# AUTOMATIC1111/stable-diffusion-webui

Measured on AMD Instinct MI355X. Metric: images/sec SD1.5 512x512 20-step Euler-a, batch 8 per GPU, higher is better.
Workload: dtype f16

## Files before the change

stable-diffusion-webui_amd/csrc/attention.hip:

```cpp
#include "common.h"
#include "prof.h"
#include <cstdlib>

namespace sdmi {

typedef float f2v __attribute__((ext_vector_type(2)));
typedef unsigned u4v __attribute__((ext_vector_type(4)));

__device__ __forceinline__ float max3f(float a, float b, float c) { return fmaxf(fmaxf(a, b), c); }
template <int NKB>
__device__ __forceinline__ float tree_max(const f16v (&sc)[NKB]) {
    constexpr int N = NKB * 16;
    float v[N];
#pragma unroll
    for (int i = 0; i < N; ++i) v[i] = sc[i >> 4][i & 15];
    int n = N;
#pragma unroll
    for (int level = 0; level < 6; ++level) {
        if (n <= 1) break;
        const int m = (n + 2) / 3;
#pragma unroll
        for (int i = 0; i < m; ++i) {
            const int a = 3 * i, b = a + 1 < n ? a + 1 : a, c = a + 2 < n ? a + 2 : a;
            v[i] = max3f(v[a], v[b], v[c]);
// ... 413 lines not shown
    h8 qf[NDC];
    {
        const half_t* qptr = p.q + ((long)b * p.N + (qok ? q : 0)) * p.ldq + h * D;
#pragma unroll
        for (int dc = 0; dc < NDC; ++dc) {
            const int d = dc * 16 + half * 8;
            h8 v = {0, 0, 0, 0, 0, 0, 0, 0};
            if (qok && d < D) v = *reinterpret_cast<const h8*>(qptr + d);
            if constexpr (FOLD) {
#pragma unroll
                for (int j = 0; j < 8; ++j) v[j] = (half_t)((float)v[j] * fold_p2(p.scale_log2));
            }
            qf[dc] = v;
        }
    }
    const half_t* kbase = p.k + (long)b * p.M * p.ldk + h * D;
    const half_t* vbase = p.vt + ((long)b * p.H + h) * D * (long)p.vt_ld;

    u4v kr[K_IT], vr[V_IT];
    auto load_k = [&](int key0) {
#pragma unroll
        for (int it = 0; it < K_IT; ++it) {
            const int idx = it * NT + tid;
            const int row = idx / KCR, c = idx - row * KCR;
            const int rr = min(key0 + row, p.M - 1);
            kr[it] = *reinterpret_cast<const u4v*>(kbase + (long)rr * p.ldk + c * 8);
        }
    };
    auto load_v = [&](int key0) {
#pragma unroll
        for (int it = 0; it < V_IT; ++it) {
            const int idx = it * NT + tid;
            const int row = idx / VCPR, c = idx - row * VCPR;
            const int col = min(key0 + c * 8, p.vt_ld - 8);
            vr[it] = *reinterpret_cast<const u4v*>(vbase + (long)min(row, D - 1) * p.vt_ld + col);
        }
    };
    char* const dump = smem + NSLOT * SLOT + K_BYTES + tid * 16;
    auto write_k = [&](char* Ks) {
#pragma unroll
        for (int it = 0; it < K_IT; ++it) {
            const int idx = it * NT + tid;
            const int row = idx / KCR, c = idx - row * KCR;
            char* dst = (KCH % NT == 0 || idx < KCH) ? Ks + row * KSTR + c * 16 : dump;
            *reinterpret_cast<u4v*>(dst) = kr[it];
        }
    };
    auto write_v = [&](char* Vs) {
#pragma unroll
        for (int it = 0; it < V_IT; ++it) {
            const int idx = it * NT + tid;
            const int row = idx / VCPR, c = idx - row * VCPR;
            char* dst = (VCH % NT == 0 || idx < VCH) ? Vs + row * VSTR + c * 16 : dump;
            *reinterpret_cast<u4v*>(dst) = vr[it];
        }
    };
    auto section_barrier = [&](bool wait_lds = true) {
        __builtin_amdgcn_sched_barrier(0);
        if (wait_lds) asm volatile("s_waitcnt lgkmcnt(0)" ::: "memory");
        __builtin_amdgcn_s_barrier();
        asm volatile("" ::: "memory");
        __builtin_amdgcn_sched_barrier(0);
    };

    const int T = (p.M + KVT - 1) / KVT;
    const int nfull = p.M / KVT;
    char* const K0s = smem + NSLOT * SLOT;

    {
        constexpr int KPAD = KCPR - KCR;
        if constexpr (KPAD > 0) {
            for (int i = tid; i < (NSLOT + 1) * KVT * KPAD; i += NT) {
                const int img = i / (KVT * KPAD), j = i - img * (KVT * KPAD);
                const int row = j / KPAD, c = KCR + j % KPAD;
                char* base = img < NSLOT ? smem + img * SLOT : K0s;
                const unsigned w0 = (FOLD && c == KCR) ? 0x00003C00u : 0u;
                *reinterpret_cast<uint4*>(base + row * KSTR + c * 16) = make_uint4(w0, 0u, 0u, 0u);
            }
        }
        if constexpr (SUMROW) {
            constexpr int PADCH = (DV - D) * VCPR;
            for (int i = tid; i < NSLOT * PADCH; i += NT) {
                const int img = i / PADCH, j = i - img * PADCH;
                const int row = D + j / VCPR, c = j % VCPR;
                const unsigned w = row == D ? 0x3C003C00u : 0u;
                *reinterpret_cast<uint4*>(smem + img * SLOT + K_BYTES + row * VSTR + c * 16) = make_uint4(w, w, w, w);
            }
        }
        load_k(0);
        write_k(K0s);
        load_v(0); load_k(KVT);
        write_v(smem + K_BYTES); write_k(smem);
        if (T > 1) {
            load_v(KVT); load_k(2 * KVT);
            write_v(smem + SLOT + K_BYTES); write_k(smem + SLOT);
        }
    }
    asm volatile("s_waitcnt lgkmcnt(0)" ::: "memory");
    __builtin_amdgcn_s_barrier();
    asm volatile("" ::: "memory");

    const int krow = (lq & 0x13) | ((lq & 4) << 1) | ((lq & 8) >> 1);
    const int ka_off = krow * KSTR + half * 16;
    const int va_off = K_BYTES + lq * VSTR + half * 16;

    f16v o[NDB], sc[NKB];
#pragma unroll
    for (int db = 0; db < NDB; ++db)
#pragma unroll
        for (int r = 0; r < 16; ++r) o[db][r] = 0.f;
#pragma unroll
    for (int kb = 0; kb < NKB; ++kb)
#pragma unroll
        for (int r = 0; r < 16; ++r) sc[kb][r] = 0.f;
    {
        h8 kaf0[NDC][NKB];
#pragma unroll
        for (int dc = 0; dc < NDC; ++dc)
#pragma unroll
            for (int kb = 0; kb < NKB; ++kb) kaf0[dc][kb] = *reinterpret_cast<const h8*>(K0s + ka_off + kb * 32 * KSTR + dc * 32);
#pragma unroll
        for (int dc = 0; dc < NDC; ++dc)
#pragma unroll
            for (int kb = 0; kb < NKB; ++kb) sc[kb] = __builtin_amdgcn_mfma_f32_32x32x16_f16(kaf0[dc][kb], qf[dc], sc[kb], 0, 0, 0);
    }
    load_v(2 * KVT); load_k(3 * KVT);

    float shift = FOLD ? 0.f : -1e30f;
    f2v l_run = {0.f, 0.f};
    const f2v sl2 = {p.scale_log2, p.scale_log2};
    [[maybe_unused]] const float fr = p.scale_log2 / fold_p2(p.scale_log2);
    [[maybe_unused]] const f2v fr2 = {fr, fr};
    h8 pb[NKB][2];
    h8 kaf[NDC][NKB], vaf[NDB][NKB][2];

    section_barrier();
    for (int i = 0; i < grp; ++i) section_barrier();
    constexpr int NB = NG;

    for (int t = 0; t < T; ++t) {
        const long long ta = stamp();
        long long tb = ta, tc = ta;
        if (t >= nfull || p.causal) {
            asm volatile("");
            int lim = p.M - t * KVT - 8 * half;
            if (p.causal) lim = min(lim, q + 1 - t * KVT - 8 * half);
#pragma unroll
            for (int kb = 0; kb < NKB; ++kb)
#pragma unroll
                for (int r = 0; r < 16; ++r)
                    if (32 * kb + 16 * (r >> 3) + (r & 7) >= lim) sc[kb][r] = -INFINITY;
        }
        float mx = tree_max<NKB>(sc);
        {
            float mlo = mx, mhi = mx;
            asm volatile("s_nop 1\n\tv_permlane32_swap_b32 %0, %1" : "+v"(mlo), "+v"(mhi));
            mx = fmaxf(mlo, mhi);
        }
        if constexpr (FOLD) {
            const bool raise = t == 0 || __builtin_amdgcn_ballot_w64(mx > 0.f) != 0;
            if (raise) {
                asm volatile("");
                const float want = shift + mx;
                const float ns = (t == 0 || mx > 0.f) ? (float)(half_t)fminf(fmaxf(want, -60000.f), 60000.f) : shift;
                const float delta = ns - shift;
                shift = ns;
                if (t > 0) {
                    const float alpha = __builtin_amdgcn_exp2f(-delta * fr);
#pragma unroll
                    for (int db = 0; db < NDB; ++db)
#pragma unroll
                        for (int r = 0; r < 16; ++r) o[db][r] *= alpha;
                    if (!SUMROW) l_run = l_run * alpha;
                }
#pragma unroll
                for (int kb = 0; kb < NKB; ++kb)
#pragma unroll
                    for (int r = 0; r < 16; ++r) sc[kb][r] -= delta;
                if (half == PHALF) qf[PDC][0] = (half_t)(-ns);
            }
        } else {
            mx *= p.scale_log2;
            const float m_new = fmaxf(shift, mx);
            const float alpha = __builtin_amdgcn_exp2f(shift - m_new);
            const bool moved = __builtin_amdgcn_ballot_w64(m_new > shift) != 0;
            shift = m_new;
            if (!SUMROW) l_run = l_run * alpha;
            if (moved) {
#pragma unroll
                for (int db = 0; db < NDB; ++db)
#pragma unroll
                    for (int r = 0; r < 16; ++r) o[db][r] *= alpha;
            }
        }
        const f2v mneg = {-shift, -shift};
        auto exp_block = [&](int kb) {
            f2v rs = {0.f, 0.f};
#pragma unroll
            for (int r = 0; r < 16; r += 2) {
                f2v e;
                if constexpr (FOLD) {
                    const f2v y = f2v{sc[kb][r], sc[kb][r + 1]} * fr2;
                    e = f2v{__builtin_amdgcn_exp2f(y.x), __builtin_amdgcn_exp2f(y.y)};
                } else {
                    const f2v s2 = {sc[kb][r], sc[kb][r + 1]};
                    const f2v y = __builtin_elementwise_fma(s2, sl2, mneg);
                    e = f2v{__builtin_amdgcn_exp2f(y.x), __builtin_amdgcn_exp2f(y.y)};
                }
                if (!SUMROW) rs += e;
                pb[kb][r >> 3][r & 7] = (half_t)e.x;
                pb[kb][r >> 3][(r & 7) + 1] = (half_t)e.y;
            }
            if (!SUMROW) l_run += rs;
        };
        auto bar = [&](int k, bool wait_lds) {
            if (!(t + 1 == T && k >= NB - grp)) section_barrier(wait_lds);
        };
        exp_block(0);
        if constexpr (NG == 3) {
            asm volatile("" :: "v"(pb[0][0]), "v"(pb[0][1]));
            tb = stamp();
            bar(0, false);
            tc = stamp();
        }
#pragma unroll
        for (int kb = 1; kb < NKB; ++kb) exp_block(kb);
        {
            const char* tile = smem + (t % NSLOT) * SLOT;
#pragma unroll
            for (int db = 0; db < NDB; ++db)
#pragma unroll
                for (int kb = 0; kb < NKB; ++kb)
#pragma unroll
                    for (int sb = 0; sb < 2; ++sb)
                        vaf[db][kb][sb] = *reinterpret_cast<const h8*>(tile + va_off + db * 32 * VSTR + (kb * 32 + sb * 16) * 2);
#pragma unroll
            for (int dc = 0; dc < NDC; ++dc)
#pragma unroll
                for (int kb = 0; kb < NKB; ++kb) kaf[dc][kb] = *reinterpret_cast<const h8*>(tile + ka_off + kb * 32 * KSTR + dc * 32);
        }
#pragma unroll
        for (int kb = 0; kb < NKB; ++kb) asm volatile("" :: "v"(pb[kb][0]), "v"(pb[kb][1]));
        const long long td = stamp();
        bar(NB - 2, false);
        const long long te = stamp();
#pragma unroll
        for (int kb = 0; kb < NKB; ++kb)
#pragma unroll
            for (int r = 0; r < 16; ++r) sc[kb][r] = 0.f;
        {
            char* slot = smem + ((t + 2) % NSLOT) * SLOT;
            write_v(slot + K_BYTES); write_k(slot);
            load_v((t + 3) * KVT); load_k((t + 4) * KVT);
        }
#pragma unroll
        for (int step = 0; step < (NDC > 2 * NKB ? NDC : 2 * NKB); ++step) {
            if (step < 2 * NKB) {
                const int kb = step >> 1, sb = step & 1;
#pragma unroll
                for (int db = 0; db < NDB; ++db) o[db] = __builtin_amdgcn_mfma_f32_32x32x16_f16(vaf[db][kb][sb], pb[kb][sb], o[db], 0, 0, 0);
            }
            if (step < NDC) {
#pragma unroll
                for (int kb = 0; kb < NKB; ++kb) sc[kb] = __builtin_amdgcn_mfma_f32_32x32x16_f16(kaf[step][kb], qf[step], sc[kb], 0, 0, 0);
            }
        }
        const long long tf = stamp();
        bar(NB - 1, true);
        if constexpr (TIMING) {
            const long long tg = stamp();
            tm[0] += tb - ta; tm[1] += tc - tb; tm[2] += td - tc; tm[3] += te - td; tm[4] += tf - te; tm[5] += tg - tf; tm[6] += 1;
        }
    }
    if constexpr (TIMING) {
        if (p.dbg && lane == 0) {
            long long* dst = p.dbg + ((long)(blockIdx.y * gridDim.x + blockIdx.x) * (4 * NG) + wave) * 8;
#pragma unroll
            for (int i = 0; i < 7; ++i) dst[i] = tm[i];
        }
    }

    float l_tot;
    if (SUMROW) l_tot = __shfl(o[L_DB][L_R], lq + 32 * L_HALF);
    else l_tot = (l_run.x + l_run.y) + __shfl_xor(l_run.x + l_run.y, 32);
    const float inv = 1.0f / l_tot;
    if (qok) {
        half_t* optr = p.out + ((long)b * p.N + q) * p.ldo + h * D;
#pragma unroll
        for (int db = 0; db < NDB; ++db) {
#pragma unroll
            for (int g = 0; g < 4; ++g) {
                const int d0 = db * 32 + g * 8 + half * 4;
                if (d0 < D) {
                    h4 v;
#pragma unroll
                    for (int e = 0; e < 4; ++e) v[e] = (half_t)(o[db][g * 4 + e] * inv);
                    *reinterpret_cast<h4*>(optr + d0) = v;
                }
            }
        }
    }
}

__global__ __launch_bounds__(64) void attn_generic_kernel(AttnP p) {
    extern __shared__ float sc[];
    const int lane = threadIdx.x;
    const int q = blockIdx.x, bh = blockIdx.y, b = bh / p.H, h = bh - b * p.H;
    const half_t* qptr = p.q + ((long)b * p.N + q) * p.ldq + h * p.D;
    const half_t* kbase = p.k + (long)b * p.M * p.ldk + h * p.D;
    const half_t* vbase = p.vt + ((long)b * p.H + h) * p.D * (long)p.vt_ld;
    float mx = -INFINITY;
    const int m_vis = p.causal ? min(p.M, q + 1) : p.M;
    for (int key = lane; key < p.M; key += 64) {
        if (key >= m_vis) { sc[key] = -INFINITY; continue; }
        const half_t* kp = kbase + (long)key * p.ldk;
        float acc = 0.f;
        for (int d = 0; d < p.D; ++d) acc = fmaf((float)qptr[d], (float)kp[d], acc);
        acc *= p.scale_log2;
        sc[key] = acc;
        mx = fmaxf(mx, acc);
    }
    for (int off = 32; off > 0; off >>= 1) mx = fmaxf(mx, __shfl_xor(mx, off));
    float sum = 0.f;
    for (int key = lane; key < p.M; key += 64) {
        const float e = exp2f(sc[key] - mx);
        sc[key] = e;
        sum += e;
    }
    for (int off = 32; off > 0; off >>= 1) sum += __shfl_xor(sum, off);
    __syncthreads();
    const float inv = 1.0f / sum;
    for (int d = lane; d < p.D; d += 64) {
        const half_t* vp = vbase + (long)d * p.vt_ld;
        float acc = 0.f;
        for (int key = 0; key < p.M; ++key) acc = fmaf(sc[key], (float)vp[key], acc);
        p.out[((long)b * p.N + q) * p.ldo + h * p.D + d] = (half_t)(acc * inv);
    }
}

__global__ __launch_bounds__(256) void transpose_v_kernel(const half_t* v, half_t* vt, int M, int C, int ldv, int Mpad) {
    __shared__ half_t tile[32][33];
    const int b = blockIdx.z;
    const int m0 = blockIdx.x * 32, c0 = blockIdx.y * 32;
    const int tx = threadIdx.x & 31, ty = threadIdx.x >> 5;
    for (int i = ty; i < 32; i += 8) {
        const int m = m0 + i, c = c0 + tx;
        tile[i][tx] = (m < M && c < C) ? v[((long)b * M + m) * ldv + c] : (half_t)0;
    }
    __syncthreads();
    for (int i = ty; i < 32; i += 8) {
        const int c = c0 + i, m = m0 + tx;
        if (c < C && m < Mpad) vt[((long)b * C + c) * Mpad + m] = tile[tx][i];
    }
}

int launch_transpose_v(const half_t* v, half_t* vt, int B, int H, int M, int D, int ldv, int Mpad, hipStream_t s) {
    const int C = H * D;
    dim3 grid(cdiv(Mpad, 32), cdiv(C, 32), B);
    hipLaunchKernelGGL(transpose_v_kernel, grid, dim3(256), 0, s, v, vt, M, C, ldv, Mpad);
    SDMI_CHECK_HIP(hipGetLastError());
    return 0;
}

unsigned long long g_attn_dbg = 0;
int g_attn_kvt = [] { const char* e = getenv("SDMI_ATTN_KVT"); return e ? atoi(e) : 0; }();

int g_attn_occ = [] { const char* e = getenv("SDMI_ATTN_OCC"); return e ? atoi(e) : 15; }();
int g_attn_tau = [] { const char* e = getenv("SDMI_ATTN_TAU"); return e ? atoi(e) : 8; }();
int g_attn_fold_min_m = [] { const char* e = getenv("SDMI_ATTN_FOLD_MIN_M"); return e ? atoi(e) : 1024; }();
int g_attn_lds_pad = 0;
int g_attn_pp_min_m = [] { const char* e = getenv("SDMI_ATTN_PP_MIN_M"); return e ? atoi(e) : 256; }();

template <int D, int KVT, int VAR = 0>
static int launch_attn_d(const AttnP& p, hipStream_t s) {
    constexpr int DK = (D + 15) / 16 * 16, DV = (D + 31) / 32 * 32;
    constexpr int SMEM = 2 * (KVT * (DK * 2 + 16) + DV * (KVT * 2 + 16));
    auto kern = attn_mfma_kernel<D, KVT, VAR>;
    static PerDeviceOnce attr;
    const int smem = SMEM + (g_attn_lds_pad > 0 ? g_attn_lds_pad : 0);
    if (attr.need(smem)) SDMI_CHECK_HIP(hipFuncSetAttribute((const void*)kern, hipFuncAttributeMaxDynamicSharedMemorySize, smem));
    dim3 grid(cdiv(p.N, 128), p.B * p.H);
    hipLaunchKernelGGL(kern, grid, dim3(256), smem, s, p);
    SDMI_CHECK_HIP(hipGetLastError());
    return 0;
}

template <int D, bool FOLD, int NG = 2, bool TIMING = false>
static int launch_attn_pp(const AttnP& p, hipStream_t s) {
    constexpr int DK = (D + 15) / 16 * 16, DV = (D + 31) / 32 * 32;
    constexpr int SMEM = 3 * (64 * (DK * 2 + 16) + DV * (64 * 2 + 16)) + 64 * (DK * 2 + 16) + NG * 256 * 16;
    auto kern = attn_pp_kernel<D, FOLD, NG, TIMING>;
    static PerDeviceOnce attr;
    if (attr.need()) SDMI_CHECK_HIP(hipFuncSetAttribute((const void*)kern, hipFuncAttributeMaxDynamicSharedMemorySize, SMEM));
    dim3 grid(cdiv(p.N, NG * 128), p.B * p.H);
    hipLaunchKernelGGL(kern, grid, dim3(NG * 256), SMEM, s, p);
    SDMI_CHECK_HIP(hipGetLastError());
    return 0;
}

int launch_attention(const AttnP& p_in, bool force_generic, hipStream_t s) {
    AttnP p = p_in;
    p.tau = (float)(g_attn_tau < 0 ? -1 : g_attn_tau > 12 ? 12 : g_attn_tau);
    SDMI_REQUIRE(p.B > 0 && p.H > 0 && p.N > 0 && p.M > 0 && p.D > 0, "empty attention");
    SDMI_REQUIRE(p.vt_ld >= (p.M + 63) / 64 * 64, "vt_ld must be >= M rounded up to 64");
    const double pf_flops = 4.0 * p.B * p.H * (double)p.N * p.M * p.D;
    const double pf_bytes = 2.0 * p.B * p.H * ((double)p.N * p.D * 2 + (double)p.M * p.D * 2);
    ProfScope ps(force_generic ? "attention_generic" : (p.M > 128 ? "attention_mfma_self" : "attention_mfma_cross"), pf_flops, pf_bytes, s);
    const bool aligned = (p.ldq % 8 == 0) && (p.ldk % 8 == 0) && (p.vt_ld % 8 == 0) && (p.ldo % 4 == 0) && (p.D % 8 == 0);
    const bool kvt128 = g_attn_kvt == 128;
    if (!force_generic && aligned) {
        if (g_attn_kvt == 96 && p.M > 64 && p.M <= 96 && !p.causal) {
            switch (p.D) {
                case 40: return launch_attn_d<40, 96, 0>(p, s);
                case 64: return launch_attn_d<64, 96>(p, s);
                case 80: return launch_attn_d<80, 96>(p, s);
                case 160: return launch_attn_d<160, 96>(p, s);
                default: break;
            }
        }
        switch (p.D) {
            case 40:
                if ((g_attn_occ == 20 || g_attn_occ == 21) && p.M >= g_attn_pp_min_m && p.N >= 256)
                    return g_attn_occ == 21 ? launch_attn_pp<40, true>(p, s) : launch_attn_pp<40, false>(p, s);
                if ((g_attn_occ == 28 || g_attn_occ == 38) && p.M >= g_attn_pp_min_m && p.N >= 384) {
                    AttnP q = p; q.dbg = (long long*)g_attn_dbg;
                    return g_attn_occ == 38 ? launch_attn_pp<40, true, 3, true>(q, s) : launch_attn_pp<40, true, 2, true>(q, s);
                }
                if ((g_attn_occ == 30 || g_attn_occ == 31) && p.M >= g_attn_pp_min_m && p.N >= 384)
                    return g_attn_occ == 31 ? launch_attn_pp<40, true, 3>(p, s) : launch_attn_pp<40, false, 3>(p, s);
                if (!(kvt128 && p.M > 64)) {
                    if (g_attn_occ == 5) return launch_attn_d<40, 64, 5>(p, s);
                    if (g_attn_occ == 15 && g_attn_fold_min_m > 0 && p.M >= g_attn_fold_min_m && p.N >= g_attn_fold_min_m && !p.causal)
                        return launch_attn_d<40, 64, 17>(p, s);
                    if (g_attn_occ == 15) return launch_attn_d<40, 64, 15>(p, s);
                    if (g_attn_occ == 16) return launch_attn_d<40, 64, 16>(p, s);
                    if (g_attn_occ == 17) return launch_attn_d<40, 64, 17>(p, s);
#ifdef SDMI_ATTN_PARTS
                    if (g_attn_occ == 10) return launch_attn_d<40, 64, 10>(p, s);
                    if (g_attn_occ == 11) return launch_attn_d<40, 64, 11>(p, s);
                    if (g_attn_occ == 12) return launch_attn_d<40, 64, 12>(p, s);
                    if (g_attn_occ == 13) return launch_attn_d<40, 64, 13>(p, s);
                    if (g_attn_occ == 14) return launch_attn_d<40, 64, 14>(p, s);
                    if (g_attn_occ == 18) { AttnP q = p; q.dbg = (long long*)g_attn_dbg; return launch_attn_d<40, 64, 18>(q, s); }
#endif
                }
                return (kvt128 && p.M > 64) ? launch_attn_d<40, 128>(p, s) : launch_attn_d<40, 64>(p, s);
            case 64:
                if ((g_attn_occ == 20 || g_attn_occ == 21) && p.M >= g_attn_pp_min_m && p.N >= 256) return launch_attn_pp<64, false>(p, s);
                return (kvt128 && p.M > 64) ? launch_attn_d<64, 128>(p, s) : launch_attn_d<64, 64>(p, s);
            case 80: return launch_attn_d<80, 64>(p, s);
            case 128: return launch_attn_d<128, 64>(p, s);
            case 160: return launch_attn_d<160, 64>(p, s);
            default: break;
        }
    }
    SDMI_REQUIRE(p.D <= 512 && p.M <= 16384, "generic attention supports D <= 512 and M <= 16384");
    static PerDeviceOnce attr;
    if (attr.need()) SDMI_CHECK_HIP(hipFuncSetAttribute((const void*)attn_generic_kernel, hipFuncAttributeMaxDynamicSharedMemorySize, 16384 * 4));
    hipLaunchKernelGGL(attn_generic_kernel, dim3(p.N, p.B * p.H), dim3(64), p.M * sizeof(float), s, p);
    SDMI_CHECK_HIP(hipGetLastError());
    return 0;
}

}
```

stable-diffusion-webui_amd/csrc/capi.cpp:

```cpp
#include "engine.h"
#include "prof.h"
#include <cstring>

namespace sdmi {
extern int g_vae_attn_rows;
int unet_forward(sdmi_engine* e, const void* x, const void* t, const void* ctx, const void* y, void* out, int io_dtype,
                 int Bn, int h, int w, int L, hipStream_t s);
int vae_decode(sdmi_engine* e, const void* z, int io_dtype, float* out, int B, int h, int w, hipStream_t s);
int vae_encode(sdmi_engine* e, const void* x, int io_dtype, float* out, int B, int H, int W, hipStream_t s);
int engine_load_unet_tensor(sdmi_engine* e, const char* key, const void* data, int dtype, int ndim, const int64_t* shape, int on_device);
int engine_load_vae_tensor(sdmi_engine* e, const char* key, const void* data, int dtype, int ndim, const int64_t* shape, int on_device);
int engine_unet_finalize(sdmi_engine* e);
int engine_clip_configure(sdmi_engine* e, int slot, const sdmi_clip_config* cfg);
int engine_clip_load_tensor(sdmi_engine* e, int slot, const char* key, const void* data, int dtype, int ndim, const int64_t* shape, int on_device);
int engine_clip_finalize(sdmi_engine* e, int slot);
int engine_clip_forward(sdmi_engine* e, int slot, const int* tokens, const float* inputs_embeds, int B, int L, int skip,
                        int apply_final_ln, float* out, float* pooled, hipStream_t s);
int engine_unet_update_weight(sdmi_engine* e, const char* key, const void* data, int dtype, int ndim, const int64_t* shape, int on_device);
int engine_vae_finalize(sdmi_engine* e);
int engine_hypernet_clear(sdmi_engine* e);
int engine_hypernet_begin(sdmi_engine* e, float multiplier);
int engine_hypernet_linear(sdmi_engine* e, int dim, int which, const void* w, const void* b, int dtype, int out_f, int in_f, int on_device);
int engine_hypernet_act(sdmi_engine* e, int dim, int which, int act);
int engine_hypernet_layernorm(sdmi_engine* e, int dim, int which, const void* g, const void* b, int dtype, int n, int on_device);
// ... 338 lines not shown
        if (f && f[0] == '1') e->force_generic = true;
        return e;
    } catch (...) {
        set_error("engine allocation failed");
        return nullptr;
    }
}
void sdmi_engine_destroy(sdmi_engine* e) { delete e; }

int sdmi_unet_configure(sdmi_engine* e, const sdmi_unet_config* cfg) {
    API_GUARD_BEGIN
    SDMI_REQUIRE(e && cfg, "null argument");
    SDMI_REQUIRE(cfg->num_levels >= 1 && cfg->num_levels <= 8, "num_levels out of range");
    SDMI_REQUIRE(cfg->model_channels % 64 == 0, "model_channels must be a multiple of 64");
    SDMI_REQUIRE(cfg->context_dim % 64 == 0, "context_dim must be a multiple of 64");
    SDMI_REQUIRE(cfg->in_channels <= 16 && cfg->out_channels <= 64, "in_channels <= 16, out_channels <= 64");
    e->unet.cfg = *cfg;
    e->unet.ready = false;
    return 0;
    API_GUARD_END
}
int sdmi_unet_load_tensor(sdmi_engine* e, const char* key, const void* data, int dtype, int ndim, const int64_t* shape,
                          int on_device) {
    API_GUARD_BEGIN
    return engine_load_unet_tensor(e, key, data, dtype, ndim, shape, on_device);
    API_GUARD_END
}
int sdmi_unet_finalize(sdmi_engine* e) {
    API_GUARD_BEGIN
    return engine_unet_finalize(e);
    API_GUARD_END
}
int sdmi_unet_update_weight(sdmi_engine* e, const char* key, const void* data, int dtype, int ndim, const int64_t* shape,
                            int on_device) {
    API_GUARD_BEGIN
    SDMI_REQUIRE(e != nullptr, "null engine");
    return engine_unet_update_weight(e, key, data, dtype, ndim, shape, on_device);
    API_GUARD_END
}
int sdmi_lora_merge(void* out, const void* w, int w_dtype, const void* up, int up_dtype, const void* down, int down_dtype,
                    int rows, int cols, int rank, float scale, void* stream) {
    API_GUARD_BEGIN
    SDMI_REQUIRE(out && w && up && down && rows > 0 && cols > 0 && rank > 0, "bad lora_merge arguments");
    return launch_lora_merge((float*)out, w, w_dtype, up, up_dtype, down, down_dtype, rows, cols, rank, scale, (hipStream_t)stream);
    API_GUARD_END
}

int sdmi_weight_hadamard(void* out, const void* w, const void* a, const void* b, float scale, int64_t n, void* stream) {
    API_GUARD_BEGIN
    SDMI_REQUIRE(out && w && a && b && n > 0, "bad arguments");
    return launch_weight_hadamard((float*)out, (const float*)w, (const float*)a, (const float*)b, scale, n, (hipStream_t)stream);
    API_GUARD_END
}

int sdmi_weight_kron(void* out, const void* w, const void* w1, const void* w2, int r1, int c1, int r2, int c2, int k, float scale,
                     void* stream) {
    API_GUARD_BEGIN
    SDMI_REQUIRE(out && w && w1 && w2 && r1 > 0 && c1 > 0 && r2 > 0 && c2 > 0 && k > 0, "bad arguments");
    return launch_weight_kron((float*)out, (const float*)w, (const float*)w1, (const float*)w2, r1, c1, r2, c2, k, scale, (hipStream_t)stream);
    API_GUARD_END
}

int sdmi_weight_ia3(void* out, const void* w, const void* v, int rows, int cols, int on_input, float scale, void* stream) {
    API_GUARD_BEGIN
    SDMI_REQUIRE(out && w && v && rows > 0 && cols > 0, "bad arguments");
    return launch_weight_ia3((float*)out, (const float*)w, (const float*)v, rows, cols, on_input, scale, (hipStream_t)stream);
    API_GUARD_END
}

int sdmi_weight_dora(void* out, const void* w, const void* delta, const void* dora_scale, int rows, int cin, int k, float mult,
                     void* stream) {
    API_GUARD_BEGIN
    SDMI_REQUIRE(out && w && delta && dora_scale && rows > 0 && cin > 0 && k > 0, "bad arguments");
    return launch_weight_dora((float*)out, (const float*)w, (const float*)delta, (const float*)dora_scale, rows, cin, k, mult,
                              (hipStream_t)stream);
    API_GUARD_END
}
int sdmi_clip_configure(sdmi_engine* e, int slot, const sdmi_clip_config* cfg) {
    API_GUARD_BEGIN
    SDMI_REQUIRE(e && cfg, "null argument");
    return engine_clip_configure(e, slot, cfg);
    API_GUARD_END
}
int sdmi_clip_load_tensor(sdmi_engine* e, int slot, const char* key, const void* data, int dtype, int ndim, const int64_t* shape,
                          int on_device) {
    API_GUARD_BEGIN
    SDMI_REQUIRE(e != nullptr, "null engine");
    return engine_clip_load_tensor(e, slot, key, data, dtype, ndim, shape, on_device);
    API_GUARD_END
}
int sdmi_clip_finalize(sdmi_engine* e, int slot) {
    API_GUARD_BEGIN
    SDMI_REQUIRE(e != nullptr, "null engine");
    return engine_clip_finalize(e, slot);
    API_GUARD_END
}
int sdmi_clip_forward(sdmi_engine* e, int slot, const void* tokens, const void* inputs_embeds, int B, int L, int skip,
                      int apply_final_ln, void* out, void* pooled, void* stream) {
    API_GUARD_BEGIN
    SDMI_REQUIRE(e != nullptr, "null engine");
    return engine_clip_forward(e, slot, (const int*)tokens, (const float*)inputs_embeds, B, L, skip, apply_final_ln, (float*)out,
                               (float*)pooled, (hipStream_t)stream);
    API_GUARD_END
}
int sdmi_unet_hypernet_clear(sdmi_engine* e) {
    API_GUARD_BEGIN
    SDMI_REQUIRE(e != nullptr, "null engine");
    return engine_hypernet_clear(e);
    API_GUARD_END
}
int sdmi_unet_hypernet_begin(sdmi_engine* e, float multiplier) {
    API_GUARD_BEGIN
    SDMI_REQUIRE(e != nullptr, "null engine");
    return engine_hypernet_begin(e, multiplier);
    API_GUARD_END
}
int sdmi_unet_hypernet_linear(sdmi_engine* e, int dim, int which, const void* w, const void* b, int dtype, int out_features, int in_features,
                              int on_device) {
    API_GUARD_BEGIN
    SDMI_REQUIRE(e != nullptr, "null engine");
    return engine_hypernet_linear(e, dim, which, w, b, dtype, out_features, in_features, on_device);
    API_GUARD_END
}
int sdmi_unet_hypernet_act(sdmi_engine* e, int dim, int which, int act) {
    API_GUARD_BEGIN
    SDMI_REQUIRE(e != nullptr, "null engine");
    return engine_hypernet_act(e, dim, which, act);
    API_GUARD_END
}
int sdmi_unet_hypernet_layernorm(sdmi_engine* e, int dim, int which, const void* gamma, const void* beta, int dtype, int n, int on_device) {
    API_GUARD_BEGIN
    SDMI_REQUIRE(e != nullptr, "null engine");
    return engine_hypernet_layernorm(e, dim, which, gamma, beta, dtype, n, on_device);
    API_GUARD_END
}
int sdmi_unet_update_vector(sdmi_engine* e, const char* key, const void* data, int dtype, int64_t n, int on_device) {
    API_GUARD_BEGIN
    SDMI_REQUIRE(e != nullptr, "null engine");
    return engine_unet_update_vector(e, key, data, dtype, n, on_device);
    API_GUARD_END
}
int sdmi_vae_configure(sdmi_engine* e, const sdmi_vae_config* cfg) {
    API_GUARD_BEGIN
    SDMI_REQUIRE(e && cfg, "null argument");
    SDMI_REQUIRE(cfg->num_levels >= 1 && cfg->num_levels <= 8 && cfg->ch % 64 == 0, "vae: ch % 64 == 0, 1..8 levels");
    SDMI_REQUIRE(cfg->z_channels <= 16 && cfg->in_channels <= 16, "vae: z_channels, in_channels <= 16");
    e->vae.cfg = *cfg;
    e->vae.ready = false;
    return 0;
    API_GUARD_END
}
int sdmi_vae_load_tensor(sdmi_engine* e, const char* key, const void* data, int dtype, int ndim, const int64_t* shape,
                         int on_device) {
    API_GUARD_BEGIN
    return engine_load_vae_tensor(e, key, data, dtype, ndim, shape, on_device);
    API_GUARD_END
}
int sdmi_vae_finalize(sdmi_engine* e) {
    API_GUARD_BEGIN
    return engine_vae_finalize(e);
    API_GUARD_END
}

int sdmi_unet_set_context(sdmi_engine* e, const void* context, int io_dtype, int Bn, int L, void* stream) {
    API_GUARD_BEGIN
    return engine_set_context(e, context, io_dtype, Bn, L, (hipStream_t)stream);
    API_GUARD_END
}
int sdmi_unet_set_context_cached(sdmi_engine* e, const void* context, int io_dtype, int Bn, int L, void* stream) {
    API_GUARD_BEGIN
    return engine_set_context(e, context, io_dtype, Bn, L, (hipStream_t)stream, true);
    API_GUARD_END
}
int sdmi_unet_forward(sdmi_engine* e, const void* x, const void* timesteps, const void* context, const void* y, void* out,
                      int io_dtype, int Bn, int h, int w, int L, void* stream) {
    API_GUARD_BEGIN
    return unet_forward(e, x, timesteps, context, y, out, io_dtype, Bn, h, w, L, (hipStream_t)stream);
    API_GUARD_END
}
int sdmi_unet_set_control(sdmi_engine* e, const void* const* tensors, const int64_t* numel, int n, int only_mid_control) {
    API_GUARD_BEGIN
    SDMI_REQUIRE(e != nullptr && n >= 0 && (n == 0 || (tensors && numel)), "null argument");
    e->control.assign(tensors, tensors + n);
    e->control_numel.assign(numel, numel + n);
    e->only_mid_control = only_mid_control != 0;
    for (int i = 0; i < n; ++i) SDMI_REQUIRE(tensors[i] != nullptr, "null control tensor");
    return 0;
    API_GUARD_END
}
int sdmi_unet_forward_ex(sdmi_engine* e, const void* x, const void* timesteps, const void* context, const void* y, void* out,
                         int io_dtype, int Bn, int h, int w, int L, int call_flags, void* stream) {
    API_GUARD_BEGIN
    SDMI_REQUIRE(e != nullptr, "null engine");
    struct Restore {
        sdmi_engine* e; bool uni, pairs, derive;
        ~Restore() { e->uniform_t = uni; e->cfg_pairs = pairs; e->auto_promises = derive; }
    } restore{e, e->uniform_t, e->cfg_pairs, e->auto_promises};
    e->uniform_t = (call_flags & SDMI_CALL_UNIFORM_T) != 0;
    e->cfg_pairs = (call_flags & SDMI_CALL_CFG_PAIRS) != 0;
    e->auto_promises = (call_flags & SDMI_CALL_DERIVE) != 0;
    return unet_forward(e, x, timesteps, context, y, out, io_dtype, Bn, h, w, L, (hipStream_t)stream);
    API_GUARD_END
}
int sdmi_vae_decode(sdmi_engine* e, const void* z, int io_dtype, void* out, int B, int h, int w, void* stream) {
    API_GUARD_BEGIN
    return vae_decode(e, z, io_dtype, (float*)out, B, h, w, (hipStream_t)stream);
    API_GUARD_END
}
int sdmi_vae_encode(sdmi_engine* e, const void* x, int io_dtype, void* out, int B, int H, int W, void* stream) {
    API_GUARD_BEGIN
    return vae_encode(e, x, io_dtype, (float*)out, B, H, W, (hipStream_t)stream);
    API_GUARD_END
}

int sdmi_rrdb_conv(const sdmi_rrdb_desc* d, void* stream) {
    API_GUARD_BEGIN
    SDMI_REQUIRE(d, "null descriptor");
    RrdbP p{};
    p.in = (const half_t*)d->in; p.w = (const half_t*)d->w; p.bias = (const float*)d->bias;
    p.r1 = (const half_t*)d->r1; p.r2 = (const half_t*)d->r2; p.out = d->out;
    p.B = d->B; p.H = d->H; p.W = d->W; p.cin = d->cin; p.lda = d->lda; p.up = d->up;
    p.ldo = d->ldo; p.n_real = d->n_real; p.ldr1 = d->ldr1; p.ldr2 = d->ldr2; p.ep = d->ep; p.store = d->store;
    p.alpha = d->alpha; p.beta = d->beta;
    return launch_rrdb_conv(p, d->nout, (hipStream_t)stream);
    API_GUARD_END
}

int64_t sdmi_esrgan_blob_floats(int num_block, int in_ch) { return esrgan_blob_floats(num_block, in_ch); }

sdmi_esrgan* sdmi_esrgan_create(sdmi_engine* e, const void* blob_f32, int64_t blob_floats, int num_block, int in_ch, int scale) {
    try {
        sdmi_esrgan* n = nullptr;
        if (esrgan_create(e, (const float*)blob_f32, blob_floats, num_block, in_ch, scale, &n) != 0) return nullptr;
        return n;
    } catch (const std::exception& ex) {
        set_error(std::string("exception: ") + ex.what());
        return nullptr;
    }
}

void sdmi_esrgan_destroy(sdmi_esrgan* h) { delete h; }

int64_t sdmi_esrgan_scratch_bytes(sdmi_esrgan* h, int B, int H, int W) { return esrgan_scratch_bytes(h, B, H, W); }

int sdmi_esrgan_run(sdmi_esrgan* h, const void* in, int in_u8, int B, int H, int W, void* out, int out_u8, void* stream) {
    API_GUARD_BEGIN
    return esrgan_run(h, in, in_u8, B, H, W, out, out_u8, (hipStream_t)stream);
    API_GUARD_END
}

int sdmi_compact_conv(const sdmi_compact_desc* d, void* stream) {
    API_GUARD_BEGIN
    SDMI_REQUIRE(d, "null descriptor");
    CompactP p{};
    p.in = (const half_t*)d->in; p.w = (const half_t*)d->w; p.bias = (const float*)d->bias; p.slope = (const float*)d->slope;
    p.base = d->base; p.out = d->out;
    p.B = d->B; p.H = d->H; p.W = d->W; p.cin = d->cin; p.lda = d->lda; p.ldo = d->ldo; p.n_real = d->n_real;
    p.ep = d->ep; p.r = d->r; p.base_u8 = d->base_u8; p.out_u8 = d->out_u8; p.grid_cap = d->grid_cap;
    return launch_compact_conv(p, (hipStream_t)stream);
    API_GUARD_END
}

int64_t sdmi_compact_blob_floats(int num_conv, int scale) { return compact_blob_floats(num_conv, scale); }

sdmi_compact* sdmi_compact_create(sdmi_engine* e, const void* blob_f32, int64_t blob_floats, int num_conv, int scale) {
    try {
        sdmi_compact* n = nullptr;
        if (compact_create(e, (const float*)blob_f32, blob_floats, num_conv, scale, &n) != 0) return nullptr;
        return n;
    } catch (const std::exception& ex) {
        set_error(std::string("exception: ") + ex.what());
        return nullptr;
    }
}

void sdmi_compact_destroy(sdmi_compact* h) { delete h; }

int64_t sdmi_compact_scratch_bytes(sdmi_compact* h, int B, int H, int W) { return compact_scratch_bytes(h, B, H, W); }

int sdmi_compact_run(sdmi_compact* h, const void* in, int in_u8, int B, int H, int W, void* out, int out_u8, void* stream) {
    API_GUARD_BEGIN
    return compact_run(h, in, in_u8, B, H, W, out, out_u8, (hipStream_t)stream);
    API_GUARD_END
}

int sdmi_debug_set(const char* name, int value) {
    API_GUARD_BEGIN
    SDMI_REQUIRE(name != nullptr, "null name");
    const std::string n(name);
    if (n == "gemm_cfg") g_force_gemm_cfg = value;
    else if (n == "gemm_shortk_cfg") g_shortk_gemm_cfg = value;
    else if (n == "vae_attn_rows") g_vae_attn_rows = value;
    else if (n == "gemm_shortk_maxk") g_shortk_max_k = value;
    else if (n == "gemm_geglu_cfg") g_geglu_gemm_cfg = value;
    else if (n == "vt_mode") g_vt_mode = value;
    else if (n == "tile_order") g_tile_order = value;
    else if (n == "conv_korder") g_conv_korder = value < 0 ? g_conv_korder_default : value;
    else if (n == "small_linear_lds") g_small_linear_lds = value;
    else if (n == "gn_fuse") g_gn_fuse = value;
    else if (n == "gn_small") g_gn_small = value;
    else if (n == "ep_wide") g_ep_wide = value;
    else if (n == "attn_kvt") g_attn_kvt = value;
    else if (n == "attn_occ") g_attn_occ = value;
    else if (n == "attn_lds_pad") g_attn_lds_pad = value;
    else if (n == "attn_fold_min_m") g_attn_fold_min_m = value;
    else if (n == "attn_tau") g_attn_tau = value;
    else if (n == "attn_dbg_lo") g_attn_dbg = (g_attn_dbg & 0xFFFFFFFF00000000ull) | (unsigned)value;
    else if (n == "attn_dbg_hi") g_attn_dbg = (g_attn_dbg & 0xFFFFFFFFull) | ((unsigned long long)(unsigned)value << 32);
    else if (n == "gemm_split") g_force_gemm_split = value;
    else if (n == "gemm_pipe") g_gemm_pipe = value < 0 ? g_gemm_pipe_default : value;
    else if (n == "gemm_lin") g_gemm_lin = value < 0 ? 1 : value;
    else if (n == "gn_apply_blocks") g_gn_apply_blocks = value < 0 ? 0 : value;
    else if (n == "gn_band_elems") g_gn_band_elems = value < 0 ? 0 : value;
    else if (n == "gemm_dbgflags") g_gemm_dbgflags = value & 0x1F00;
    else if (n == "gemm_dbg_lo") g_gemm_dbg = (g_gemm_dbg & 0xFFFFFFFF00000000ull) | (unsigned)value;
    else if (n == "gemm_dbg_hi") g_gemm_dbg = (g_gemm_dbg & 0xFFFFFFFFull) | ((unsigned long long)(unsigned)value << 32);
    else { set_error("unknown debug knob " + n); return 1; }
    return 0;
    API_GUARD_END
}

int sdmi_debug_set_str(const char* name, const char* value) {
    API_GUARD_BEGIN
    SDMI_REQUIRE(name != nullptr, "null name");
    if (std::string(name) == "gemm_override") {
        SDMI_REQUIRE(gemm_set_override(value) == 0, "gemm_override: expected M,N,K,taps,kind:cfg:split;...");
        return 0;
    }
    set_error(std::string("unknown debug knob ") + name);
    return 1;
    API_GUARD_END
}

int sdmi_profile_begin(void) {
    prof_begin();
    return 0;
}
int sdmi_profile_end(char* json_out, int capacity) {
    const std::string s = prof_end();
    if (!json_out || capacity <= (int)s.size()) {
        set_error("profile buffer too small");
        return 1;
    }
    std::memcpy(json_out, s.c_str(), s.size() + 1);
    return 0;
}

int64_t sdmi_engine_arena_bytes(sdmi_engine* e) { return e ? (int64_t)e->arena.cap : 0; }

int sdmi_engine_set_option(sdmi_engine* e, const char* name, int value) {
    API_GUARD_BEGIN
    SDMI_REQUIRE(e && name, "null argument");
    const std::string n(name);
    if (n == "force_generic") e->force_generic = value != 0;
    else if (n == "glds") e->use_glds = value != 0;
    else if (n == "trace") { e->trace = value != 0; e->taps.clear(); }
    else if (n == "tiling") e->tiling = value != 0;
    else if (n == "uniform_t") e->uniform_t = value != 0;
    else if (n == "cfg_pairs") e->cfg_pairs = value != 0;
    else if (n == "auto_promises") e->auto_promises = value != 0;
    else if (n == "ln_fold") e->ln_fold = value;
    else if (n == "fuse_rows") e->fuse_rows = value;
    else if (n == "residual_fp32") e->residual_fp32 = value != 0;
    else if (n == "arena_reuse") e->arena_reuse = value;
    else if (n == "streams") { if (value < 1 || value > 8) { sdmi::set_error("streams must be 1..8"); return 1; } e->n_streams = value; }
    else if (n == "vae_range_extend") e->vae_stream_scale = value ? 1.0f / 64.0f : 1.0f;
    else { set_error("unknown option " + n); return 1; }
    return 0;
    API_GUARD_END
}

int sdmi_engine_tap_count(sdmi_engine* e) { return e ? (int)e->taps.size() : 0; }
int sdmi_engine_tap_info(sdmi_engine* e, int index, char* name_out, int capacity, int64_t* dims_bhwc) {
    API_GUARD_BEGIN
    SDMI_REQUIRE(e && name_out && dims_bhwc && index >= 0 && index < (int)e->taps.size(), "bad tap index / null argument");
    const auto& t = e->taps[index];
    SDMI_REQUIRE((int)t.name.size() < capacity, "tap name buffer too small");
    std::memcpy(name_out, t.name.c_str(), t.name.size() + 1);
    dims_bhwc[0] = t.B; dims_bhwc[1] = t.H; dims_bhwc[2] = t.W; dims_bhwc[3] = t.C;
    return 0;
    API_GUARD_END
}
int sdmi_engine_tap_read(sdmi_engine* e, int index, void* out_f16_nhwc, void* stream) {
    API_GUARD_BEGIN
    SDMI_REQUIRE(e && out_f16_nhwc && index >= 0 && index < (int)e->taps.size(), "bad tap index / null argument");
    const auto& t = e->taps[index];
    SDMI_CHECK_HIP(hipMemcpyAsync(out_f16_nhwc, t.ptr, (size_t)t.B * t.H * t.W * t.C * sizeof(half_t), hipMemcpyDeviceToDevice,
                                  (hipStream_t)stream));
    return 0;
    API_GUARD_END
}

}
```

stable-diffusion-webui_amd/csrc/common.h:

```cpp
#pragma once
#include <hip/hip_runtime.h>
#include <stdint.h>
#include <string>

typedef _Float16 half_t;
typedef _Float16 h8 __attribute__((ext_vector_type(8)));
typedef _Float16 h4 __attribute__((ext_vector_type(4)));
typedef _Float16 h2 __attribute__((ext_vector_type(2)));
typedef float f4 __attribute__((ext_vector_type(4)));
typedef float f16v __attribute__((ext_vector_type(16)));

namespace sdmi {

#ifndef SDMI_GELU_SIG
#define SDMI_GELU_SIG 1
#endif
__device__ __forceinline__ float geglu_gate(float val, float g) {
    const float gc = fminf(fmaxf(g, -10.0f), 10.0f);
    const float g2 = gc * gc;
    float p = fmaf(1.01426306e-3f, g2, -0.106775724f);
    p = fmaf(p, g2, -2.30112135f);
    const float e = __builtin_amdgcn_exp2f(p * gc);
    return (val * g) * __builtin_amdgcn_rcpf(1.0f + e);
}

void set_error(const std::string& msg);
const char* get_error();

#define SDMI_CHECK_HIP(expr)                                                                       \
    do {                                                                                           \
        hipError_t _e = (expr);                                                                    \
        if (_e != hipSuccess) {                                                                    \
            ::sdmi::set_error(std::string(#expr) + ": " + hipGetErrorString(_e));                  \
            return 1;                                                                              \
        }                                                                                          \
    } while (0)

#define SDMI_REQUIRE(cond, msg)                                                                    \
    do {                                                                                           \
        if (!(cond)) {                                                                             \
            ::sdmi::set_error(std::string("requirement failed: ") + #cond + " — " + (msg));        \
            return 1;                                                                              \
        }                                                                                          \
    } while (0)

static inline int cdiv(int64_t a, int64_t b) { return (int)((a + b - 1) / b); }

struct PerDeviceOnce {
    int level[64] = {};
    bool need(int want = 1) {
        int d = 0;
        if (hipGetDevice(&d) != hipSuccess) d = 0;
        d &= 63;
        if (level[d] >= want) return false;
        level[d] = want;
        return true;
    }
};

constexpr int kZeroPageHalfs = 16384;
const half_t* zero_page();

struct GemmP {
    const half_t* a0;
    const half_t* a1;
    const half_t* w;
    const float* bias;
    const float* rowbias;
    const half_t* resid;
    void* out;
    const half_t* zero;
    int c0, c1, cin;
    int lda0, lda1;
    int Hi, Wi, Ho, Wo;
    int taps, stride, pad, up;
    int M, N, K;
    int ldo, ldr;
    int ldw;
    int ldrb;
    int rows_per_batch;
    int n_real;
    int n_valid;
    int flags;
    float alpha;
    long a_bs, w_bs, o_bs, r_bs;
    float* splitk_ws;
    int splitk;
    int splitk_steps;
    long long* dbg;
    float* stats_out;
    int stats_cpg;
    int stats_nchunk;
    int korder;
    int tile_order;
    float bias_scale;
    const int* gate;
    const float* ln_stats;
    const float* ln_s;
    int ln_np;
    float ln_inv_c, ln_eps;
    float* lnp_out;
    int lnp_np;
};

enum { EP_OUT_F32 = 1, EP_GEGLU = 2, EP_NCHW = 4, EP_BIAS_ROW = 8,
       EP_QUICK_GELU = 16, EP_GELU = 32,
       EP_TRANSPOSE = 64,
       EP_WRAP = 128,
       EP_DBG_NO_BAR_A = 0x100, EP_DBG_NO_BAR_B = 0x200, EP_DBG_NO_GLDS = 0x400, EP_DBG_NO_VMWAIT = 0x800,
       EP_DBG_NO_DSREAD = 0x1000,
       EP_LNFOLD = 0x4000,
       EP_HILO = 0x8000,
       EP_NARROW = 0x2000
     };

__host__ __device__ inline half_t* gemm_out_lo(const GemmP& p) {
    return (p.flags & EP_HILO) ? reinterpret_cast<half_t*>(const_cast<float*>(p.ln_stats)) : nullptr;
}
__host__ __device__ inline const half_t* gemm_resid_lo(const GemmP& p) { return (p.flags & EP_HILO) ? reinterpret_cast<const half_t*>(p.ln_s) : nullptr; }

int launch_gemm(const GemmP& p, int batch, bool force_generic, bool use_glds, hipStream_t s, int* stats_nchunk_out = nullptr,
                int* lnp_np_out = nullptr);
extern int g_ep_wide;
extern int g_small_linear_lds;
extern int g_gn_small;
extern int g_gn_fuse;
size_t gemm_splitk_ws_bytes(int M, int N, int K, int batch);
int gemm_set_override(const char* spec);
extern int g_force_gemm_cfg;
extern int g_shortk_gemm_cfg;
extern int g_shortk_max_k;
extern int g_geglu_gemm_cfg;
extern int g_conv_korder;
extern int g_conv_korder_default;
extern int g_tile_order;
extern int g_vt_mode;
extern long g_gn_band_elems;
extern int g_gn_apply_blocks;
extern int g_gemm_lin;
extern int g_gemm_pipe;
extern int g_gemm_pipe_default;
extern int g_force_gemm_split;
extern int g_attn_kvt;
extern int g_attn_occ;
extern int g_attn_lds_pad;
extern int g_attn_fold_min_m;
extern int g_attn_tau;
extern unsigned long long g_attn_dbg;
extern int g_gemm_dbgflags;
extern unsigned long long g_gemm_dbg;

struct AttnP {
    const half_t* q;
    const half_t* k;
    const half_t* vt;
    half_t* out;
    int B, H, N, M, D;
    int ldq, ldk, vt_ld, ldo;
    float scale_log2;
    int causal;
    long long* dbg;
    float tau;
};
int launch_attention(const AttnP& p, bool force_generic, hipStream_t s);
int launch_transpose_v(const half_t* v, half_t* vt, int B, int H, int M, int D, int ldv, int Mpad, hipStream_t s);

bool rowchain_supports(int C);
size_t rowchain_ff_pack_bytes(int C, int hidden);
int launch_rowchain_ff_pack(const half_t* w1, const float* b1, const half_t* w2, void* packs, int C, int hidden, bool permuted,
                            hipStream_t s);
int launch_rowchain_ff(const half_t* x, half_t* out, const float* gamma, const float* beta, const void* packs, const float* bias_out,
                       long rows, int C, int hidden, float eps, hipStream_t s);

enum { RRDB_EP_NONE = 0, RRDB_EP_LRELU = 1,
       RRDB_EP_RES1 = 2,
       RRDB_EP_RES2 = 3 };
enum { RRDB_ST_F16 = 0, RRDB_ST_F32_NCHW = 1, RRDB_ST_U8_HWC = 2 };
struct RrdbP {
    const half_t* in;
    const half_t* w;
    const float* bias;
    const half_t* r1;
    const half_t* r2;
    void* out;
    const half_t* zero;
    int B, H, W;
    int cin, lda, ldw, up;
    int ldo, n_real, ldr1, ldr2;
    int ep, store;
    float alpha, beta;
    long long M;
};
int launch_rrdb_conv(const RrdbP& p, int nout, hipStream_t s);
int launch_rrdb_input(const void* in, int u8, half_t* out, int B, int C, int H, int W, int f, int cpad, hipStream_t s);

enum { COMPACT_EP_NONE = 0, COMPACT_EP_PRELU = 1,
       COMPACT_EP_TAIL = 2 };
struct CompactP {
    const half_t* in;
    const half_t* w;
    const float* bias;
    const float* slope;
    const void* base;
    void* out;
    const half_t* zero;
    int B, H, W;
    int cin, lda, ldo, n_real;
    int ep, r, base_u8, out_u8;
    int grid_cap;
    int tiles_x, tiles_y;
    int tiles;
};
int launch_compact_conv(const CompactP& p, hipStream_t s);

int launch_groupnorm(const half_t* x0, const half_t* x1, int c0, int c1, const float* gamma, const float* beta,
                     half_t* out, int B, int HW, int groups, float eps, bool silu, float* ws, hipStream_t s, int pre_nchunk = 0,
                     const half_t* x0_lo = nullptr, const half_t* x1_lo = nullptr);
int64_t groupnorm_ws_bytes(int B, int HW, int groups);
int launch_layernorm(const half_t* x, const float* gamma, const float* beta, half_t* out, int64_t rows, int C,
                     float eps, hipStream_t s, const half_t* x_lo = nullptr);
int launch_ln_rowstats(const half_t* x, float* stats, int64_t rows, int C, float eps, hipStream_t s);
int launch_ln_fold_weights(const half_t* w, const float* gamma, const float* beta, const float* bias, half_t* wf, float* s_out,
                           float* c_out, int n_rows, int K, int C, hipStream_t s);

int launch_philox(float* out, int64_t n, uint64_t seed, uint32_t offset, hipStream_t s);
int launch_cfg_prepare(const float* x, const float* c_in, void* xin, int out_dtype, int B, int reps, int64_t chw, hipStream_t s);
int launch_slerp(float* out, const float* low, const float* high, float val, int C, int H, int W, float* scratch, hipStream_t s);
int launch_weight_hadamard(float* out, const float* w, const float* a, const float* b, float scale, int64_t n, hipStream_t s);
int launch_weight_kron(float* out, const float* w, const float* w1, const float* w2, int r1, int c1, int r2, int c2, int k, float scale,
                       hipStream_t s);
int launch_weight_ia3(float* out, const float* w, const float* v, int rows, int cols, int on_input, float scale, hipStream_t s);
int launch_weight_dora(float* out, const float* w, const float* delta, const float* dora_scale, int rows, int cin, int k, float mult,
                       hipStream_t s);
int launch_cfg_prepare_concat(const float* x, const float* c_in, const float* cond, void* xin, int out_dtype, int B, int reps,
                              int C, int Cc, int64_t hw, unsigned zero_reps, hipStream_t s);
int launch_cfg_combine(const float* x, const float* eps, const float* c_out, float cond_scale, int mode,
                       const float* mask, const float* nmask, const float* init_latent, float* den, int B,
                       int64_t chw, hipStream_t s);
int launch_euler_step(float* x, const float* den, const float* noise, float sigma, float sigma_down, float sigma_up,
                      float s_noise, int64_t n, hipStream_t s);
int launch_dpmpp2m_step(float* x, const float* den, const float* old, float ratio, float em1, float c1, float c2,
                        int64_t n, hipStream_t s);
int launch_ddim_step(float* x, const float* e, const float* noise, float* pred_x0, float a_t, float a_prev,
                     float sigma_t, float somat, int64_t n, hipStream_t s);
int launch_axpby(float* y, const float* x, float a, const float* z, float b, int64_t n, hipStream_t s);
int launch_dpm_error(const float* lo, const float* hi, const float* prev, float atol, float rtol, float* partial256, int64_t n,
                     hipStream_t s);
int launch_lincomb(float* out, const float* const* terms, const float* coefs, int n_terms, int64_t n, hipStream_t s);
int launch_lora_merge(float* out, const void* w, int w_dtype, const void* up, int up_dtype, const void* down, int down_dtype,
                      int rows, int cols, int rank, float scale, hipStream_t s);
int launch_clip_embed(const int* tokens, const void* tok_emb, int tok_dtype, const float* pos_emb, const float* inputs_embeds,
                      half_t* out, int B, int L, int C, int vocab, hipStream_t s);
int launch_clip_pool(const int* tokens, const half_t* hidden, float* pooled, int B, int L, int C, hipStream_t s);
int launch_latent_resize(const float* in, float* out, int planes, int hi, int wi, int ho, int wo, int mode, hipStream_t s);
int launch_cfg_combine_affine(const float* x, const float* out, const float* c_out, const float* c_skip, float cond_scale,
                              const float* mask, const float* nmask, const float* init_latent, float* den, int B, int64_t chw,
                              hipStream_t s);
int launch_act_f16(half_t* x, int64_t n, int kind, hipStream_t s);
int launch_axpy_f16(half_t* y, const half_t* x, const half_t* h, float a, int64_t n, hipStream_t s);
int launch_silu_f32(const float* x, float* y, int64_t n, hipStream_t s);
int launch_mask_blend(float* x, const float* init, const float* mask, const float* nmask, int64_t n, hipStream_t s);
int launch_image_to_u8(const float* img, uint8_t* out, int B, int C, int H, int W, hipStream_t s);

int launch_nchw_to_nhwc(const void* x, int dtype, half_t* out, int B, int C, int HW, int cpad, float scale,
                        const float* mix_w, const float* mix_b, hipStream_t s, bool lo_ch = false);
int launch_add_nchw_residual(const half_t* src, const half_t* src_lo, const void* ctrl, int dtype, half_t* dst, half_t* dst_lo, int B, int C,
                             int HW, hipStream_t s);
int launch_copy_out(const float* src, void* dst, int dtype, int64_t n, hipStream_t s);
int launch_convert_to_f16(const void* src, int dtype, half_t* dst, int64_t n, hipStream_t s);
int launch_convert_to_f32(const void* src, int dtype, float* dst, int64_t n, hipStream_t s);
int launch_ctx_compare(const void* src, int dtype, const half_t* cached, int B, int L, int Lpad, int C, int* gate, hipStream_t s);
int launch_ctx_update_gated(const void* src, int dtype, half_t* cached, int B, int L, int Lpad, int C, const int* gate, hipStream_t s);
int launch_timestep_embedding(const void* t, int dtype, float* out, int B, int dim, hipStream_t s);
int launch_small_linear(const float* a, const half_t* w, const float* bias, const float* add, float* out, int B,
                        int N, int K, int lda, int ldo, bool silu_in, bool silu_out, hipStream_t s);
int launch_softmax_rows(const float* in, half_t* out, int64_t rows, int cols, int ldi, int ldo, hipStream_t s);
int launch_pack_conv_weight(const void* w, int dtype, half_t* out, int O, int I, int kh, int kw, int O_pad,
                            int I_pad, int geglu, hipStream_t s);
int launch_pack_bias(const void* b, int dtype, float* out, int O, int O_pad, int geglu, hipStream_t s);

}
```

Measured before the change: 21.59.

## Add register-resident cross-attention kernel keeping K/V in VGPRs across query blocks

```diff
diff --git a/stable-diffusion-webui_amd/csrc/attention.hip b/stable-diffusion-webui_amd/csrc/attention.hip
--- a/stable-diffusion-webui_amd/csrc/attention.hip
+++ b/stable-diffusion-webui_amd/csrc/attention.hip
@@ -739,6 +739,161 @@
     }
 }
 
+__device__ __forceinline__ void permlane32_swap(float& x, float& y) {
+    asm volatile("s_nop 1\n\tv_permlane32_swap_b32 %0, %1" : "+v"(x), "+v"(y));
+}
+
+template <int D, int HWMAX>
+__global__ __launch_bounds__(HWMAX * 64) void attn_ctx_kernel(AttnP p, int qb_per_wg) {
+    constexpr int DK = (D + 15) / 16 * 16, NDC = DK / 16;
+    constexpr int DV = (D + 31) / 32 * 32, NDB = DV / 32;
+    constexpr int NKB = 3;
+    static_assert(D % 8 == 0, "head size must be a multiple of 8");
+    const int lane = threadIdx.x & 63;
+    const int wave = __builtin_amdgcn_readfirstlane(threadIdx.x >> 6);
+    const int half = lane >> 5, lq = lane & 31;
+    const int b = blockIdx.z, h = blockIdx.y * (blockDim.x >> 6) + wave;
+    if (h >= p.H) return;
+    const h8 zero8 = {0, 0, 0, 0, 0, 0, 0, 0};
+
+    h8 kaf[NDC][NKB], vaf[NDB][NKB][2];
+    {
+        const int krow = (lq & 0x13) | ((lq & 4) << 1) | ((lq & 8) >> 1);
+        const half_t* kbase = p.k + (long)b * p.M * p.ldk + h * D + half * 8;
+#pragma unroll
+        for (int kb = 0; kb < NKB; ++kb) {
+            const half_t* krp = kbase + (long)min(kb * 32 + krow, p.M - 1) * p.ldk;
+#pragma unroll
+            for (int dc = 0; dc < NDC; ++dc) {
+                h8 v = zero8;
+                if (DK == D || dc * 16 + half * 8 < D) v = *reinterpret_cast<const h8*>(krp + dc * 16);
+                kaf[dc][kb] = v;
+            }
+        }
+        const half_t* vbase = p.vt + ((long)b * p.H + h) * D * (long)p.vt_ld + half * 8;
+#pragma unroll
+        for (int db = 0; db < NDB; ++db) {
+            const half_t* vrp = vbase + (long)min(db * 32 + lq, D - 1) * p.vt_ld;
+#pragma unroll
+            for (int kb = 0; kb < NKB; ++kb)
+#pragma unroll
+                for (int sb = 0; sb < 2; ++sb) {
+                    h8 v = *reinterpret_cast<const h8*>(vrp + kb * 32 + sb * 16);
+                    if (kb == 2) {
+#pragma unroll
+                        for (int e = 0; e < 8; ++e)
+                            if (64 + sb * 16 + half * 8 + e >= p.M) v[e] = (half_t)0;
+                    }
+                    vaf[db][kb][sb] = v;
+                }
+        }
+    }
+
+    const int nblk = (p.N + 31) >> 5;
+    const int blk0 = blockIdx.x * qb_per_wg;
+    const int nb = min(qb_per_wg, nblk - blk0);
+    const half_t* qbase = p.q + (long)b * p.N * p.ldq + h * D + half * 8;
+    half_t* obase = p.out + (long)b * p.N * p.ldo + h * D + half * 8;
+    auto load_q = [&](int blk, h8 (&dst)[NDC]) {
+        const half_t* src = qbase + (long)min(blk * 32 + lq, p.N - 1) * p.ldq;
+#pragma unroll
+        for (int dc = 0; dc < NDC; ++dc) dst[dc] = *reinterpret_cast<const h8*>(src + dc * 16 - ((DK > D && dc * 16 + half * 8 >= D) ? half * 8 : 0));
+    };
+    auto take = [&](h8 v, int dc) -> h8 {
+        asm volatile("" : "+v"(v));
+        return (DK > D && dc * 16 + half * 8 >= D) ? zero8 : v;
+    };
+    const int lim = p.M - 64 - 8 * half;
+    const f2v sl2 = {p.scale_log2, p.scale_log2};
+
+    h8 qf[NDC], qn[NDC];
+    load_q(blk0, qf);
+#pragma unroll
+    for (int dc = 0; dc < NDC; ++dc) qf[dc] = take(qf[dc], dc);
+    for (int i = 0; i < nb; ++i) {
+        const int blk = blk0 + i;
+        if (i + 1 < nb) load_q(blk + 1, qn);
+        __builtin_amdgcn_sched_barrier(0);
+
+        f16v sc[NKB];
+#pragma unroll
+        for (int kb = 0; kb < NKB; ++kb)
+#pragma unroll
+            for (int r = 0; r < 16; ++r) sc[kb][r] = 0.f;
+#pragma unroll
+        for (int dc = 0; dc < NDC; ++dc)
+#pragma unroll
+            for (int kb = 0; kb < NKB; ++kb) sc[kb] = __builtin_amdgcn_mfma_f32_32x32x16_f16(kaf[dc][kb], qf[dc], sc[kb], 0, 0, 0);
+#pragma unroll
+        for (int r = 0; r < 16; ++r)
+            if (16 * (r >> 3) + (r & 7) >= lim) sc[2][r] = -INFINITY;
+
+        float mx = tree_max<NKB>(sc);
+        {
+            float mlo = mx, mhi = mx;
+            permlane32_swap(mlo, mhi);
+            mx = fmaxf(mlo, mhi) * p.scale_log2;
+        }
+        const f2v mneg = {-mx, -mx};
+        f2v rs = {0.f, 0.f};
+        h8 pb[NKB][2];
+#pragma unroll
+        for (int kb = 0; kb < NKB; ++kb)
+#pragma unroll
+            for (int r = 0; r < 16; r += 2) {
+                const f2v s2 = {sc[kb][r], sc[kb][r + 1]};
+                const f2v y = __builtin_elementwise_fma(s2, sl2, mneg);
+                const f2v e = {__builtin_amdgcn_exp2f(y.x), __builtin_amdgcn_exp2f(y.y)};
+                rs += e;
+                pb[kb][r >> 3][r & 7] = (half_t)e.x;
+                pb[kb][r >> 3][(r & 7) + 1] = (half_t)e.y;
+            }
+
+        f16v o[NDB];
+#pragma unroll
+        for (int db = 0; db < NDB; ++db) {
+#pragma unroll
+            for (int r = 0; r < 16; ++r) o[db][r] = 0.f;
+#pragma unroll
+            for (int kb = 0; kb < NKB; ++kb)
+#pragma unroll
+                for (int sb = 0; sb < 2; ++sb) o[db] = __builtin_amdgcn_mfma_f32_32x32x16_f16(vaf[db][kb][sb], pb[kb][sb], o[db], 0, 0, 0);
+        }
+        float inv;
+        {
+            float llo = rs.x + rs.y, lhi = llo;
+            permlane32_swap(llo, lhi);
+            inv = 1.0f / (llo + lhi);
+        }
+
+        if (i + 1 < nb) {
+#pragma unroll
+            for (int dc = 0; dc < NDC; ++dc) qf[dc] = take(qn[dc], dc);
+        }
+
+        const int q = blk * 32 + lq;
+        half_t* optr = obase + (long)min(q, p.N - 1) * p.ldo;
+#pragma unroll
+        for (int db = 0; db < NDB; ++db)
+#pragma unroll
+            for (int gp = 0; gp < 2; ++gp) {
+                if (db * 32 + gp * 16 >= D) continue;
+                h4 lo4, hi4;
+#pragma unroll
+                for (int e = 0; e < 4; ++e) {
+                    lo4[e] = (half_t)(o[db][gp * 8 + e] * inv);
+                    hi4[e] = (half_t)(o[db][gp * 8 + 4 + e] * inv);
+                }
+                f2v a = __builtin_bit_cast(f2v, lo4), c = __builtin_bit_cast(f2v, hi4);
+                float a0 = a.x, a1 = a.y, c0 = c.x, c1 = c.y;
+                permlane32_swap(a0, c0);
+                permlane32_swap(a1, c1);
+                const f4 w = {a0, a1, c0, c1};
+                if (q < p.N && db * 32 + gp * 16 + half * 8 < D) *reinterpret_cast<f4*>(optr + db * 32 + gp * 16) = w;
+            }
+    }
+}
+
 __global__ __launch_bounds__(64) void attn_generic_kernel(AttnP p) {
     extern __shared__ float sc[];
     const int lane = threadIdx.x;
@@ -835,6 +990,21 @@
     return 0;
 }
 
+int g_attn_ctx = [] { const char* e = getenv("SDMI_ATTN_CTX"); return e ? atoi(e) : 1; }();
+
+template <int D, int HWMAX>
+static int launch_attn_ctx(const AttnP& p, hipStream_t s) {
+    int hw = p.H < HWMAX ? p.H : HWMAX;
+    while (p.H % hw) --hw;
+    const int nblk = cdiv(p.N, 32), groups = p.B * (p.H / hw);
+    const int want = groups >= 256 ? 1 : 256 / groups;
+    const int qb = g_attn_ctx > 1 ? (g_attn_ctx < nblk ? g_attn_ctx : nblk) : cdiv(nblk, want < nblk ? want : nblk);
+    dim3 grid(cdiv(nblk, qb), p.H / hw, p.B);
+    hipLaunchKernelGGL((attn_ctx_kernel<D, HWMAX>), grid, dim3(hw * 64), 0, s, p, qb);
+    SDMI_CHECK_HIP(hipGetLastError());
+    return 0;
+}
+
 int launch_attention(const AttnP& p_in, bool force_generic, hipStream_t s) {
     AttnP p = p_in;
     p.tau = (float)(g_attn_tau < 0 ? -1 : g_attn_tau > 12 ? 12 : g_attn_tau);
@@ -852,6 +1022,14 @@
                 case 64: return launch_attn_d<64, 96>(p, s);
                 case 80: return launch_attn_d<80, 96>(p, s);
                 case 160: return launch_attn_d<160, 96>(p, s);
+                default: break;
+            }
+        }
+        if (g_attn_ctx != 0 && g_attn_kvt != 96 && p.M > 64 && p.M <= 96 && !p.causal && p.vt_ld >= 128 && p.ldo % 8 == 0) {
+            switch (p.D) {
+                case 40: return launch_attn_ctx<40, 8>(p, s);
+                case 64: return launch_attn_ctx<64, 5>(p, s);
+                case 80: return launch_attn_ctx<80, 4>(p, s);
                 default: break;
             }
         }
diff --git a/stable-diffusion-webui_amd/csrc/capi.cpp b/stable-diffusion-webui_amd/csrc/capi.cpp
--- a/stable-diffusion-webui_amd/csrc/capi.cpp
+++ b/stable-diffusion-webui_amd/csrc/capi.cpp
@@ -664,6 +664,7 @@
     else if (n == "ep_wide") g_ep_wide = value;
     else if (n == "attn_kvt") g_attn_kvt = value;
     else if (n == "attn_occ") g_attn_occ = value;
+    else if (n == "attn_ctx") g_attn_ctx = value;
     else if (n == "attn_lds_pad") g_attn_lds_pad = value;
     else if (n == "attn_fold_min_m") g_attn_fold_min_m = value;
     else if (n == "attn_tau") g_attn_tau = value;
diff --git a/stable-diffusion-webui_amd/csrc/common.h b/stable-diffusion-webui_amd/csrc/common.h
--- a/stable-diffusion-webui_amd/csrc/common.h
+++ b/stable-diffusion-webui_amd/csrc/common.h
@@ -143,6 +143,7 @@
 extern int g_force_gemm_split;
 extern int g_attn_kvt;
 extern int g_attn_occ;
+extern int g_attn_ctx;
 extern int g_attn_lds_pad;
 extern int g_attn_fold_min_m;
 extern int g_attn_tau;
```

New measurement: 21.72, median of 5. About the same (+0.6%).
